# Hyungi-Lee/Scale-Mixtures-of-Neural-Network-Gaussian-Processes

Measured on AMD Instinct MI355X. Metric: kernel-build + Cholesky wallclock (ms) and GFLOP/s at N=16384, 4-layer relu NNGP, higher is better.
Workload: dtype f32; 1 GPU; C4: SPR.loss = NNGP kernel build + jittered Cholesky + Gaussian LML, N=16384 d=3072 L=4 relu; N=16384, d=3072, layers=4, act=relu, parallelism=single GPU

## Files before the change

### include/smnngp.h

```cpp
#ifndef SMNNGP_H
#define SMNNGP_H

#include <stddef.h>
#include <stdint.h>

#ifdef __cplusplus
extern "C" {
#endif

typedef struct smn_ctx smn_ctx;

enum { SMN_OK = 0, SMN_EINVAL = -1, SMN_EHIP = -2, SMN_ENOMEM = -3, SMN_ENOTSUP = -4, SMN_ECOMM = -5 };
enum { SMN_F32 = 0, SMN_F64 = 1 };
enum { SMN_ACT_RELU = 0, SMN_ACT_ERF = 1 };
enum { SMN_GET_NNGP = 1, SMN_GET_NTK = 2 };
enum { SMN_FILL_FULL = 0, SMN_FILL_LOWER = 1 };
enum { SMN_NET_MLP = 0, SMN_NET_DENSE_RESNET = 1 };

int smn_version(void);
int smn_device_count(int* n);
int smn_ctx_create(int device_id, smn_ctx** out);
int smn_ctx_destroy(smn_ctx* ctx);
int smn_last_error(smn_ctx* ctx, char* buf, size_t n);
int smn_synchronize(smn_ctx* ctx);
// ... 62 lines not shown

int smn_trsm(smn_ctx* ctx, int dtype, const void* l_d, int64_t n, int64_t ldl,
             void* b_d, int64_t nrhs, int64_t ldb, int trans);
int smn_transpose(smn_ctx* ctx, int dtype, void* dst_d, int64_t ldd, const void* src_d, int64_t lds, int64_t rows,
                  int64_t cols);

int smn_lml(smn_ctx* ctx, int dtype, void* k_d, int64_t n, int64_t ldk, const void* y_d,
            double eps_abs, double df, double scale, double* logpdf_h, double* quad_h,
            double* logdet_h, int* info_h);

int smn_predict(smn_ctx* ctx, int dtype, void* kj_d, int64_t n, int64_t t, int64_t ldk,
                const void* y_d, int64_t c, double ridge_rel, double ridge_abs,
                void* mean_d, void* cov_d, int64_t ldcov, double* quad_h, double* logdet_h, int* info_h);

int smn_spr_loss(smn_ctx* ctx, int dtype, int net, int act, int num_hiddens,
                 double w_std, double b_std, double last_w_std,
                 const void* x_d, int64_t n, int64_t ldx, int64_t d, const void* y_d,
                 double eps_abs, double df, double scale,
                 double* logpdf_h, double* quad_h, double* logdet_h, int* info_h);
int smn_spr_predict(smn_ctx* ctx, int dtype, int net, int act, int num_hiddens,
                    double w_std, double b_std, double last_w_std,
                    const void* x_d, int64_t n, int64_t ldx, const void* xt_d, int64_t t, int64_t ldxt,
                    int64_t d, const void* y_d, int64_t c, double ridge_rel, double ridge_abs,
                    void* mean_d, void* cov_d, int64_t ldcov,
                    double* quad_h, double* logdet_h, int* info_h);

int smn_spr_loss_batch(smn_ctx* ctx, int dtype, int net, int act, int num_hiddens, int nprob,
                       const double* w_std, const double* b_std, const double* last_w_std,
                       const void* x_d, int64_t n, int64_t ldx, int64_t d, const void* y_d,
                       const double* eps_abs, const double* df, const double* scale,
                       double* logpdf_h, double* quad_h, double* logdet_h, int* info_h);
int smn_debug_batch_bytes(smn_ctx* ctx, size_t bytes);
int smn_debug_split_build(smn_ctx* ctx, int on);
int smn_debug_gram_cache(smn_ctx* ctx, int on);
int smn_gram_cache_stats(smn_ctx* ctx, int64_t* hits, int64_t* misses, size_t* bytes);
int smn_debug_panel_passes(smn_ctx* ctx, int max_passes);
int smn_spr_predict_batch(smn_ctx* ctx, int dtype, int net, int act, int num_hiddens, int nprob,
                          const double* w_std, const double* b_std, const double* last_w_std,
                          const void* x_d, int64_t n, int64_t ldx, const void* xt_d, int64_t t, int64_t ldxt,
                          int64_t d, const void* y_d, int64_t c, const double* ridge_rel, const double* ridge_abs,
                          void* mean_d, void* cov_d, int64_t ldcov, void* var_d,
                          double* quad_h, double* logdet_h, int* info_h);

int smn_mixture_nll(smn_ctx* ctx, int dtype, int nprob, int64_t t, const void* mean_d, const void* var_d,
                    const double* quad_h, const double* logdet_h, const int* skip_h, const double* y_test_h,
                    double y_mean, double y_std, int64_t n, int nmix, int nsamples, const double* sample_q_h,
                    const double* ratio_h, double* tnll_h);

int smn_lml_grad_terms(smn_ctx* ctx, int dtype, int net, int act, int num_hiddens,
                       double w_std, double b_std, double last_w_std,
                       const void* k0_d, int64_t n, int64_t ldk0, const void* q_d,
                       const void* neg_kinv_d, int64_t ldkinv, const void* alpha_d,
                       double coef, double terms_h[4]);
int smn_spr_loss_grad(smn_ctx* ctx, int dtype, int net, int act, int num_hiddens,
                      double w_std, double b_std, double last_w_std,
                      const void* x_d, int64_t n, int64_t ldx, int64_t d, const void* y_d,
                      double eps_abs, double df, double scale,
                      double* quad_h, double* logdet_h, int* info_h, double terms_h[4]);
int smn_spr_loss_grad_batch(smn_ctx* ctx, int dtype, int net, int act, int num_hiddens, int nprob,
                            const double* w_std, const double* b_std, const double* last_w_std,
                            const void* x_d, int64_t n, int64_t ldx, int64_t d, const void* y_d,
                            const double* eps_abs, const double* df, const double* scale,
                            double* quad_h, double* logdet_h, int* info_h, double* terms_h);

#define SMN_CNN_GRAD_MAX_PIXELS 1024
int smn_kernel_cnn_grad_terms(smn_ctx* ctx, int dtype, int act, int num_hiddens,
// ... 71 lines not shown
```

### scale-mixtures-of-neural-network-gaussian-processes_amd/_lib.py

```python
from __future__ import annotations

import ctypes as C
import os

import numpy as np

_HERE = os.path.dirname(os.path.abspath(__file__))
LIB_PATH = os.environ.get("SMNNGP_LIB") or os.path.join(_HERE, "libsmnngp.so")

OK, EINVAL, EHIP, ENOMEM, ENOTSUP, ECOMM = 0, -1, -2, -3, -4, -5
F32, F64 = 0, 1
ACT = {"relu": 0, "erf": 1}
GET_NNGP, GET_NTK = 1, 2
FILL_FULL, FILL_LOWER = 0, 1
NET_MLP, NET_DENSE_RESNET = 0, 1


class SmnError(RuntimeError):
    def __init__(self, code, msg):
        super().__init__("libsmnngp error %d: %s" % (code, msg))
        self.code = code


def _load():
# ... 22 lines not shown
    "smn_free": [_vp, _vp],
    "smn_memset": [_vp, _vp, _i, _sz],
    "smn_memcpy_h2d": [_vp, _vp, _vp, _sz],
    "smn_memcpy_d2h": [_vp, _vp, _vp, _sz],
    "smn_memcpy_d2d": [_vp, _vp, _vp, _sz],
    "smn_memcpy2d_h2d": [_vp, _vp, _sz, _vp, _sz, _sz, _sz],
    "smn_memcpy2d_d2h": [_vp, _vp, _sz, _vp, _sz, _sz, _sz],
    "smn_timer_start": [_vp],
    "smn_timer_stop_ms": [_vp, _pd],
    "smn_profile_enable": [_vp, _i],
    "smn_profile_read": [_vp, _i, _pd, _pi],
    "smn_profile_flops": [_vp, _i, _pd],
    "smn_kernel_mlp": [_vp, _i, _i, _i, _i, _d, _d, _d, _vp, _i64, _i64, _vp, _i64, _i64, _i64, _i, _i, _vp, _vp, _i64],
    "smn_kernel_mlp_rows": [_vp, _i, _i, _i, _i, _d, _d, _d, _vp, _i64, _i64, _i64, _i64, _i64, _i, _vp, _vp, _i64],
    "smn_kernel_mlp_lower_rows": [_vp, _i, _i, _i, _i, _d, _d, _d, _vp, _i64, _i64, _i64, _i64, _i64, _i, _vp, _vp, _i64],
    "smn_kernel_mlp_shard": [_vp, _i, _i, _i, _i, _d, _d, _d, _vp, _i64, _i64, _i64, _i, _i, _i64, _i, _vp, _vp],
    "smn_gram": [_vp, _i, _vp, _i64, _i64, _vp, _i64, _i64, _i64, _vp, _i64, _vp, _vp],
    "smn_recursion": [_vp, _i, _i, _i, _i, _d, _d, _d, _vp, _i64, _i64, _i64, _vp, _vp, _i, _i, _vp, _vp, _i64],
    "smn_kernel_cnn": [_vp, _i, _i, _i, _d, _d, _d, _vp, _i64, _vp, _i64, _i64, _i64, _i64, _i, _vp, _i64],
    "smn_kernel_conv_resnet": [_vp, _i, _i, _i, _d, _d, _d, _vp, _i64, _vp, _i64, _i64, _i64, _i64, _i, _vp, _i64],
    "smn_cholesky": [_vp, _i, _vp, _i64, _i64, _i64, _i64, _d, _d, _pi, _pd],
    "smn_trsm": [_vp, _i, _vp, _i64, _i64, _vp, _i64, _i64, _i],
    "smn_transpose": [_vp, _i, _vp, _i64, _vp, _i64, _i64, _i64],
    "smn_lml": [_vp, _i, _vp, _i64, _i64, _vp, _d, _d, _d, _pd, _pd, _pd, _pi],
    "smn_predict": [_vp, _i, _vp, _i64, _i64, _i64, _vp, _i64, _d, _d, _vp, _vp, _i64, _pd, _pd, _pi],
    "smn_spr_loss": [_vp, _i, _i, _i, _i, _d, _d, _d, _vp, _i64, _i64, _i64, _vp, _d, _d, _d, _pd, _pd, _pd, _pi],
    "smn_spr_predict": [_vp, _i, _i, _i, _i, _d, _d, _d, _vp, _i64, _i64, _vp, _i64, _i64, _i64, _vp, _i64, _d, _d,
                        _vp, _vp, _i64, _pd, _pd, _pi],
    "smn_spr_loss_batch": [_vp, _i, _i, _i, _i, _i, _pd, _pd, _pd, _vp, _i64, _i64, _i64, _vp, _pd, _pd, _pd, _pd, _pd, _pd, _pi],
    "smn_spr_predict_batch": [_vp, _i, _i, _i, _i, _i, _pd, _pd, _pd, _vp, _i64, _i64, _vp, _i64, _i64, _i64, _vp, _i64, _pd, _pd,
                              _vp, _vp, _i64, _vp, _pd, _pd, _pi],
    "smn_debug_batch_bytes": [_vp, _sz],
    "smn_debug_split_build": [_vp, C.c_int],
    "smn_debug_gram_cache": [_vp, C.c_int],
    "smn_gram_cache_stats": [_vp, C.POINTER(C.c_int64), C.POINTER(C.c_int64), C.POINTER(C.c_size_t)],
    "smn_debug_panel_passes": [_vp, C.c_int],
    "smn_mixture_nll": [_vp, _i, _i, _i64, _vp, _vp, _pd, _pd, _pi, _pd, _d, _d, _i64, _i, _i, _pd, _pd, _pd],
    "smn_comm_unique_id": [C.c_char_p],
    "smn_lml_grad_terms": [_vp, _i, _i, _i, _i, _d, _d, _d, _vp, _i64, _i64, _vp, _vp, _i64, _vp, _d, _pd],
    "smn_spr_loss_grad": [_vp, _i, _i, _i, _i, _d, _d, _d, _vp, _i64, _i64, _i64, _vp, _d, _d, _d, _pd, _pd, _pi, _pd],
    "smn_spr_loss_grad_batch": [_vp, _i, _i, _i, _i, _i, _pd, _pd, _pd, _vp, _i64, _i64, _i64, _vp, _pd, _pd, _pd, _pd, _pd, _pi, _pd],
    "smn_kernel_cnn_grad_terms": [_vp, _i, _i, _i, _d, _d, _d, _vp, _i64, _i64, _i64, _i64, _vp, _i64, _vp, _d, _pd],
    "smn_spr_cnn_loss_grad": [_vp, _i, _i, _i, _d, _d, _d, _vp, _i64, _i64, _i64, _i64, _vp, _d, _d, _d, _pd, _pd, _pi, _pd],
    "smn_kernel_conv_diag": [_vp, _i, _i, _i, _i, _d, _d, _d, _vp, _i64, _i64, _i64, _i64, _vp],
    "smn_svsp_moments": [_vp, _i, _vp, _vp, _vp, _vp, _vp, _i64, _i64, _i64, _d, _vp, _vp, _pi, _pi64],
    "smn_mc_softmax": [_vp, _i, _vp, _vp, _pi, _i64, _i64, _i64, _d, C.c_uint64, _i64, _vp, _vp, _vp, _vp],
    "smn_rng_variates": [_vp, _i, C.c_uint64, _d, _i64, _i64, _i64, _i64, _vp],
    "smn_rng_variates_ddf": [_vp, _i, C.c_uint64, _d, _i64, _i64, _i64, _i64, _vp, _vp],
    "smn_svsp_head_grad": [_vp, _i, _vp, _vp, _pi, _i64, _i64, _i64, _d, _d, C.c_uint64, _i64, _vp, _vp, _pd, _vp, _vp, _pd, _pd, _pi],
    "smn_svsp_elbo_grad": [_vp, _i, _vp, _i64, _i64, _i64, _i64, _vp, _vp, _d, _d, _d, _pi, _i64, _d, _d, C.c_uint64, _i64, _vp, _vp,
                           _pd, _pd, _vp, _vp, _pd, _pd, _pd, _pd, _vp, _i64, _pi],
    "smn_debug_philox": [_vp, C.POINTER(C.c_uint32), C.POINTER(C.c_uint32), C.POINTER(C.c_uint32)],
    "smn_comm_init": [_vp, _i, _i, C.c_char_p],
    "smn_comm_destroy": [_vp],
    "smn_allgather": [_vp, _i, _i, _vp, _vp, _i64],
    "smn_unpack_lower_blocks": [_vp, _i, _vp, _i64, _i, _i64, _vp, _i64],
    "smn_lml_from_blocks": [_vp, _i, _vp, _i64, _i, _i64, _vp, _d, _d, _d, _pd, _pd, _pd, _pi],
    "smn_comm_info": [_vp, _pi, _pi],
    "smn_shard_begin": [_vp, _i, _i64, _d],
    "smn_kernel_mlp_shard_cols": [_vp, _i, _i, _i, _i, _d, _d, _d, _vp, _i64, _i64, _i64, _i, _i, _i, _pi64, _i, _vp, _vp],
    "smn_shard_exchange_cols": [_vp, _i, _vp, _vp, _i64, _i, _i, _pi64, _i],
    "smn_shard_exchange_cols_to": [_vp, _i, _vp, _vp, _i64, _i, _i, _pi64, _i, _vp, _i64],
    "smn_shard_scatter_cols": [_vp, _i, _vp, _i64, _i, _i, _pi64, _i, _vp, _i64],
    "smn_shard_wait": [_vp],
    "smn_lml_from_shards": [_vp, _i, _i64, _vp, _d, _d, _pd, _pd, _pd, _pi],
    "smn_debug_delay": [_vp, _i, _i64],
# ... 200 lines not shown
```

### scale-mixtures-of-neural-network-gaussian-processes_amd/csrc/api.hip

```cpp
#include <climits>

#include "internal.hpp"

int smn_allow_lds(smn_ctx* ctx, const void* kernel, size_t lds) {
  size_t& have = ctx->max_lds[kernel];
  if (lds <= have) return SMN_OK;
  SMN_HIP(ctx, hipFuncSetAttribute(kernel, hipFuncAttributeMaxDynamicSharedMemorySize, (int)lds));
  have = lds;
  return SMN_OK;
}

static int sync_side_streams(smn_ctx* ctx) {
  if (ctx->stream_comm) SMN_HIP(ctx, hipStreamSynchronize(ctx->stream_comm));
  if (ctx->stream_scatter) SMN_HIP(ctx, hipStreamSynchronize(ctx->stream_scatter));
  if (ctx->stream_bulk) SMN_HIP(ctx, hipStreamSynchronize(ctx->stream_bulk));
  return SMN_OK;
}

int smn_workspace(smn_ctx* ctx, int slot, size_t bytes, void** out) {
  if (slot < 0 || slot >= smn_ctx::kSlots) return smn_fail(ctx, SMN_EINVAL, "bad workspace slot");
  if (ctx->ws_bytes[slot] < bytes) {
    if (slot == 2) {
      ctx->shard_a = nullptr;
      ctx->arrivals.clear();
// ... 231 lines not shown
extern "C" int smn_ctx_create(int device_id, smn_ctx** out) {
  if (!out) return SMN_EINVAL;
  *out = nullptr;
  int cnt = 0;
  if (hipGetDeviceCount(&cnt) != hipSuccess || cnt <= 0 || device_id < 0 || device_id >= cnt) return SMN_EHIP;
  if (hipSetDevice(device_id) != hipSuccess) return SMN_EHIP;
  smn_ctx* c = new smn_ctx();
  c->device = device_id;
  if (const char* e = getenv("SMN_XCD_MAP")) c->xcd_map = e[0] == '1';
  if (const char* e = getenv("SMN_SUPER")) c->super_panel = atol(e);
  if (const char* e = getenv("SMN_SUPER_WIDE_ROWS")) c->super_wide_rows = atol(e);
  if (const char* e = getenv("SMN_PANEL_LEAF")) c->panel_leaf = e[0] != '0';
  {
    hipDeviceProp_t prop;
    if (hipGetDeviceProperties(&prop, device_id) == hipSuccess && prop.multiProcessorCount > 0)
      c->num_cu = prop.multiProcessorCount;
  }
  int prio_lo = 0, prio_hi = 0;
  (void)hipDeviceGetStreamPriorityRange(&prio_lo, &prio_hi);
  auto masked_stream = [&](hipStream_t* st, int lo, int hi) -> bool {
    uint32_t mask[8] = {0, 0, 0, 0, 0, 0, 0, 0};
    for (int b = lo; b < hi && b < 256; ++b) mask[b >> 5] |= 1u << (b & 31);
    return hipExtStreamCreateWithCUMask(st, 8, mask) == hipSuccess;
  };
  const bool main_ok = hipStreamCreateWithPriority(&c->stream, hipStreamNonBlocking, prio_hi) == hipSuccess;
  if (const char* e = getenv("SMN_CHAIN_CUS")) c->chain_cus = atoi(e);
  if (const char* e = getenv("SMN_CHAIN_MIN_N")) c->chain_min_n = atol(e);
  if (c->chain_cus > 0 && c->chain_cus < c->num_cu) {
    if (!masked_stream(&c->stream_bulk, c->chain_cus, c->num_cu)) c->stream_bulk = nullptr;
  }
  bool ok = main_ok &&
            hipEventCreateWithFlags(&c->ev_a, hipEventDisableTiming) == hipSuccess &&
            hipEventCreateWithFlags(&c->ev_b, hipEventDisableTiming) == hipSuccess &&
            hipEventCreateWithFlags(&c->ev_c0, hipEventDisableTiming) == hipSuccess &&
            hipEventCreateWithFlags(&c->ev_c1, hipEventDisableTiming) == hipSuccess &&
            hipStreamCreateWithPriority(&c->stream_comm, hipStreamNonBlocking, prio_hi) == hipSuccess &&
            hipStreamCreateWithPriority(&c->stream_scatter, hipStreamNonBlocking, prio_hi) == hipSuccess &&
            hipEventCreate(&c->ev_t0) == hipSuccess && hipEventCreate(&c->ev_t1) == hipSuccess &&
            hipMalloc(reinterpret_cast<void**>(&c->d_scal), 64 * sizeof(double)) == hipSuccess &&
            hipMalloc(reinterpret_cast<void**>(&c->d_info), 16 * sizeof(int)) == hipSuccess &&
            hipHostMalloc(reinterpret_cast<void**>(&c->h_mail), smn_ctx::kMailDoubles * sizeof(double), hipHostMallocMapped) == hipSuccess &&
            hipHostGetDevicePointer(reinterpret_cast<void**>(&c->d_mail), c->h_mail, 0) == hipSuccess;
  if (!ok) {
    smn_ctx_destroy(c);
    return SMN_EHIP;
  }
  c->h_mail[smn_ctx::kMailGram] = 0.0;
  *out = c;
  return SMN_OK;
}

extern "C" int smn_ctx_destroy(smn_ctx* c) {
  if (!c) return SMN_OK;
  (void)hipSetDevice(c->device);
  if (c->stream_bulk) (void)hipStreamSynchronize(c->stream_bulk);
  if (c->stream_comm) (void)hipStreamSynchronize(c->stream_comm);
  if (c->stream_scatter) (void)hipStreamSynchronize(c->stream_scatter);
  if (c->stream) (void)hipStreamSynchronize(c->stream);
  if (c->comm) smn_comm_destroy(c);
  gram_cache_drop(c, true);
  if (c->gram.word) (void)hipFree(c->gram.word);
  for (int i = 0; i < smn_ctx::kSlots; ++i)
    if (c->ws[i]) (void)hipFree(c->ws[i]);
  for (hipEvent_t e : c->prof_ev) (void)hipEventDestroy(e);
  if (c->d_scal) (void)hipFree(c->d_scal);
  if (c->d_info) (void)hipFree(c->d_info);
  if (c->h_mail) (void)hipHostFree(c->h_mail);
  if (c->ev_a) (void)hipEventDestroy(c->ev_a);
  if (c->ev_b) (void)hipEventDestroy(c->ev_b);
  if (c->ev_s0) (void)hipEventDestroy(c->ev_s0);
  if (c->ev_corner) (void)hipEventDestroy(c->ev_corner);
  if (c->tile_list) (void)hipFree(c->tile_list);
  if (c->ev_c0) (void)hipEventDestroy(c->ev_c0);
  if (c->ev_c1) (void)hipEventDestroy(c->ev_c1);
  if (c->stream_comm) (void)hipStreamDestroy(c->stream_comm);
  if (c->stream_scatter) (void)hipStreamDestroy(c->stream_scatter);
  for (hipEvent_t e : c->ev_pool) (void)hipEventDestroy(e);
  if (c->ev_t0) (void)hipEventDestroy(c->ev_t0);
  if (c->ev_t1) (void)hipEventDestroy(c->ev_t1);
  if (c->stream) (void)hipStreamDestroy(c->stream);
  if (c->stream_bulk) (void)hipStreamDestroy(c->stream_bulk);
  delete c;
  return SMN_OK;
}

extern "C" int smn_last_error(smn_ctx* ctx, char* buf, size_t n) {
  if (!ctx || !buf || n == 0) return SMN_EINVAL;
  snprintf(buf, n, "%s", ctx->err.c_str());
  return SMN_OK;
}

extern "C" int smn_synchronize(smn_ctx* ctx) {
  if (!ctx) return SMN_EINVAL;
  SMN_ENTER(ctx);
  SMN_HIP(ctx, hipStreamSynchronize(ctx->stream));
  return SMN_OK;
}

extern "C" int smn_malloc(smn_ctx* ctx, size_t bytes, void** dptr) {
  if (!ctx || !dptr) return SMN_EINVAL;
  SMN_ENTER(ctx);
  *dptr = nullptr;
// ... 118 lines not shown
```

### scale-mixtures-of-neural-network-gaussian-processes_amd/csrc/cholesky.hip

```cpp
#include <climits>
#include <cstdlib>
#include <type_traits>
#include <vector>

#include "gemm_nt.hpp"
#include "internal.hpp"
#include "panel_leaf.hpp"

namespace {

constexpr int PB = 128;
constexpr int MP = 8;
constexpr int kQuarterTileMax = 256;
constexpr int kHalfTileMax = 384;
constexpr int kPersistMaxK = 512;
constexpr int kPanelSmallRows = 4096;
constexpr int kPanelSmallXR = 16;
constexpr int64_t kSuperWide = 2048;
constexpr int64_t kOuterWide = 512;
constexpr int64_t kF0FirstTiles = 2000;

template <typename T>
struct PanelCfg;
#ifndef SMN_PANEL_XR
#define SMN_PANEL_XR 128
#endif
template <>
struct PanelCfg<float> {
  static constexpr int XR = SMN_PANEL_XR;
  static constexpr int LD = PB + 4;
};
template <>
struct PanelCfg<double> {
  static constexpr int XR = 16;
  static constexpr int LD = PB + 2;
};
template <typename T>
struct PanelMma;
template <>
struct PanelMma<float> {
  static constexpr int TM = 16, ACC = 4, KSTEP = 16, NK = 4;
  using acc_t = f32x4;
  using vec_t = f32x4;
  static __device__ __forceinline__ int frag_row(int lane) { return lane & 15; }
  static __device__ __forceinline__ int frag_k(int lane) { return (lane >> 4) * 4; }
  static __device__ __forceinline__ void mma1(acc_t& c, float a, float b) {
    c = __builtin_amdgcn_mfma_f32_16x16x4f32(a, b, c, 0, 0, 0);
  }
  static __device__ __forceinline__ int acc_row(int lane, int i) { return 4 * (lane >> 4) + i; }
  static __device__ __forceinline__ int acc_col(int lane) { return lane & 15; }
};
template <>
struct PanelMma<double> {
// ... 857 lines not shown
  }
}

template <typename T>
__global__ void diag_trace_kernel(const T* __restrict__ a, int64_t lda, int64_t n, double* __restrict__ out) {
  __shared__ double red[256];
  double s = 0.0;
  for (int64_t i = threadIdx.x; i < n; i += 256) s += (double)a[i * lda + i];
  red[threadIdx.x] = s;
  __syncthreads();
  for (int o = 128; o > 0; o >>= 1) {
    if ((int)threadIdx.x < o) red[threadIdx.x] += red[threadIdx.x + o];
    __syncthreads();
  }
  if (threadIdx.x == 0) *out = red[0];
}

template <typename T>
__global__ void diag_shift_kernel(T* __restrict__ a, int64_t lda, int64_t n, double jitter_abs, double ridge_rel,
                                  const double* __restrict__ trace) {
  const int64_t i = (int64_t)blockIdx.x * blockDim.x + threadIdx.x;
  if (i >= n) return;
  const double sh = jitter_abs + (ridge_rel != 0.0 ? ridge_rel * (*trace) / (double)n : 0.0);
  a[i * lda + i] = (T)((double)a[i * lda + i] + sh);
}

__global__ void init_scalars_kernel(double* logdet, int* info) {
  *logdet = 0.0;
  *info = INT_MAX;
}

template <typename T>
int launch_update(smn_ctx* ctx, const FactorCall& f, hipStream_t st, T* a, int64_t lda, int64_t r0, int64_t c0, int64_t k0,
                  int64_t K, int64_t tiles_m, int64_t tiles_n, int lower, int tag = -1) {
  if (tiles_m <= 0 || tiles_n <= 0 || K <= 0) return SMN_OK;
  if (tag < 0) tag = lower ? 1 : 0;
  if (f.id0 >= 0) {
    const int64_t id0 = f.id0, id1 = f.id1, r_end = r0 + tiles_m * kTile;
    const int64_t act = std::min(id1, id0 + (k0 + K + kTile - 1) / kTile * kTile);
    if (act < id1 && r_end > act) {
      FactorCall live = f;
      live.id0 = live.id1 = -1;
      if (r0 < act) SMN_TRY(launch_update<T>(ctx, live, st, a, lda, r0, c0, k0, K, (act - r0) / kTile, tiles_n, lower, tag));
      if (r_end > id1) {
        const int64_t tb = (r_end - id1) / kTile;
        const int64_t nb = lower == 1 ? (act - c0) / kTile : tiles_n;
        SMN_TRY(launch_update<T>(ctx, live, st, a, lda, id1, c0, k0, K, tb, nb, 0, tag));
        if (lower == 1) SMN_TRY(launch_update<T>(ctx, live, st, a, lda, id1, id1, k0, K, tb, tb, 1, tag));
      }
      return SMN_OK;
    }
  }
  if (lower == 2 && tiles_n >= tiles_m) {
    lower = 1;
    tiles_n = tiles_m;
  }
  UpdArgs<T> u{a, lda, r0, c0, k0, (int)K, (int)tiles_n, lower, 0, TileMap::make(tiles_m, tiles_n, lower == 1),
               f.batch_logdet ? f.batch_stride : 0};
  const unsigned gy = (unsigned)(f.batch_logdet ? f.batch : 1);
  int64_t nt = lower == 1   ? tiles_m * (tiles_m + 1) / 2
               : lower == 2 ? tiles_n * (tiles_n + 1) / 2 + (tiles_m - tiles_n) * tiles_n
                            : tiles_m * tiles_n;
  ctx->prof_flops[tag ? PROF_TRAIL : PROF_STRIP] += 2.0 * kTile * kTile * (double)K * (double)nt * gy;
  if (ctx->xcd_map && nt >= 512 && lower != 2) {
    u.use_map = 1;
    nt = u.map.grid;
  }
  const size_t lds = MainTile<T>::LDS_BYTES;
  if constexpr (sizeof(T) == 4) {
    const int cus = (st == ctx->stream_bulk && st != nullptr) ? ctx->num_cu - ctx->chain_cus : ctx->num_cu;
    if (tag == 1 && lower && !u.use_map && gy == 1 && nt > 2 * cus && K <= kPersistMaxK) {
      const size_t plds = TileNT<T, kTile, kTile, 2>::LDS_BYTES;
      ProfScope ps(ctx, PROF_TRAIL, st);
      hipLaunchKernelGGL(trail_kernel<T>, dim3((unsigned)(2 * cus)), dim3(256), plds, st, u, (int)nt);
      SMN_CHECK_LAUNCH(ctx);
      return SMN_OK;
    }
  }
  if (!u.use_map && nt <= kQuarterTileMax) {
    ProfScope ps(ctx, tag ? PROF_TRAIL : PROF_STRIP, st);
    constexpr size_t qlds = TileNT<T, 64, 64, SMN_STAGES>::LDS_BYTES;
    if (tag) {
      auto kern = update_kernel<T, 1, 64, 64>;
      hipLaunchKernelGGL(kern, dim3((unsigned)(4 * nt), gy), dim3(256), qlds, st, u);
    } else {
      auto kern = update_kernel<T, 0, 64, 64>;
      hipLaunchKernelGGL(kern, dim3((unsigned)(4 * nt), gy), dim3(256), qlds, st, u);
    }
    SMN_CHECK_LAUNCH(ctx);
    return SMN_OK;
  }
  if (!u.use_map && nt <= kHalfTileMax) {
    const int64_t nh = lower == 1   ? tiles_m * (tiles_m + 1)
                       : lower == 2 ? tiles_n * (tiles_n + 1) + 2 * (tiles_m - tiles_n) * tiles_n
                                    : 2 * tiles_m * tiles_n;
    ProfScope ps(ctx, tag ? PROF_TRAIL : PROF_STRIP, st);
    constexpr size_t hlds = TileNT<T, 64, kTile, SMN_STAGES>::LDS_BYTES;
    if (tag) {
      auto kern = update_kernel<T, 1, 64>;
      hipLaunchKernelGGL(kern, dim3((unsigned)nh, gy), dim3(256), hlds, st, u);
    } else {
      auto kern = update_kernel<T, 0, 64>;
      hipLaunchKernelGGL(kern, dim3((unsigned)nh, gy), dim3(256), hlds, st, u);
    }
// ... 127 lines not shown
  }
  SMN_CHECK_LAUNCH(ctx);
  hipStream_t sb = (n_total >= ctx->chain_min_n && ctx->stream_bulk) ? ctx->stream_bulk : nullptr;
  const int64_t W = sb ? kOuterWide : 2 * PB;
  int64_t S = ctx->super_panel / W * W;
  if (S < W) S = W;
  int64_t Swide = kSuperWide;
  if (Swide < S) Swide = S;
  const bool noschur = f.noschur && n_factor < n_total;
  const bool arriving = f.n_arrivals > 0;
  std::vector<char> seen_main, seen_bulk;
  if (arriving) {
    seen_main.assign(f.n_arrivals, 0);
    seen_bulk.assign(f.n_arrivals, 0);
  }
  bool first_need = true;
  auto need_columns = [&](hipStream_t s, int64_t col_hi) -> int {
    if (!arriving) return SMN_OK;
    std::vector<char>& seen = (s == st) ? seen_main : seen_bulk;
    bool any = false;
    for (size_t i = 0; i < f.n_arrivals; ++i)
      if (!seen[i] && f.arrivals[i].col_begin < col_hi) any = true;
    if (!any) return SMN_OK;
    ProfScope ps(ctx, first_need ? PROF_EXPOSED : PROF_STALL, s);
    first_need = false;
    for (size_t i = 0; i < f.n_arrivals; ++i)
      if (!seen[i] && f.arrivals[i].col_begin < col_hi) {
        SMN_HIP(ctx, hipStreamWaitEvent(s, f.arrivals[i].ev, 0));
        seen[i] = 1;
      }
    return SMN_OK;
  };
  auto width = [&](int64_t c0) { return (sb && n_total - c0 >= ctx->super_wide_rows) ? Swide : S; };
  for (int64_t s0 = 0, s_stop = 0; s0 < n_factor; s0 = s_stop) {
    const int64_t Sc = width(s0);
    const int64_t s_end = (n_factor - s0 < Sc) ? n_factor : s0 + Sc;
    s_stop = s_end;
    for (int64_t j0 = s0; j0 < s_end; j0 += W) {
      const int64_t w = (s_end - j0 < W) ? s_end - j0 : W;
      for (int64_t js = j0; js < j0 + w; js += PB) {
        SMN_TRY(need_columns(st, js + PB));
        if (js > j0)
          SMN_TRY(launch_update<T>(ctx, f, st, a, lda, js, js, j0, js - j0, (n_total - js) / kTile, 1, 0));
        SMN_TRY(launch_panel<T>(ctx, f, st, a, lda, js, n_total, 0));
      }
      const int64_t j1 = j0 + w;
      if (j1 < s_end) SMN_TRY(need_columns(st, s_end));
      if (j1 < s_end)
        SMN_TRY(launch_update<T>(ctx, f, st, a, lda, j1, j1, j0, w, (n_total - j1) / kTile, (s_end - j1) / kTile, 2));
    }
    if (s_end >= n_total) break;
    const int64_t K = s_end - s0;
    if (!sb) {
      SMN_TRY(need_columns(st, n_total));
      const int64_t tm = (n_total - s_end) / kTile;
      if (!noschur) SMN_TRY(launch_update<T>(ctx, f, st, a, lda, s_end, s_end, s0, K, tm, tm, 1));
      else if (n_factor > s_end) SMN_TRY(launch_update<T>(ctx, f, st, a, lda, s_end, s_end, s0, K, tm, (n_factor - s_end) / kTile, 2));
      continue;
    }
    const int64_t Sn = width(s_end);
    const int64_t s_next = s_end >= n_factor ? s_end : ((n_factor - s_end < Sn) ? n_factor : s_end + Sn);
    const int64_t tm1 = n_total > s_next ? (n_total - s_next) / kTile : 0;
    const int64_t tn1 = noschur ? (n_factor > s_next ? (n_factor - s_next) / kTile : 0) : tm1;
    const bool f0_first = tn1 * (tn1 + 1) / 2 + (tm1 - tn1) * tn1 <= kF0FirstTiles;
    if (!f0_first) {
      SMN_HIP(ctx, hipEventRecord(ctx->ev_a, st));
      SMN_HIP(ctx, hipStreamWaitEvent(sb, ctx->ev_a, 0));
    }
    if (bulk.side) SMN_HIP(ctx, hipStreamWaitEvent(st, ctx->ev_b, 0));
    if (s_next > s_end) SMN_TRY(need_columns(st, s_next));
    if (s_next > s_end)
      SMN_TRY(launch_update<T>(ctx, f, st, a, lda, s_end, s_end, s0, K, (n_total - s_end) / kTile, (s_next - s_end) / kTile, 2));
    if (f0_first) {
      SMN_HIP(ctx, hipEventRecord(ctx->ev_a, st));
      SMN_HIP(ctx, hipStreamWaitEvent(sb, ctx->ev_a, 0));
    }
    if (n_total > s_next && tn1 > 0) {
      const int64_t tm = (n_total - s_next) / kTile;
      bulk.side = sb;
      SMN_TRY(need_columns(sb, n_total));
      if (!noschur) {
        SMN_TRY(launch_update<T>(ctx, f, sb, a, lda, s_next, s_next, s0, K, tm, tm, 1));
      } else {
        SMN_TRY(launch_update<T>(ctx, f, sb, a, lda, s_next, s_next, s0, K, tn1, tn1, 1));
        if (tm > tn1) SMN_TRY(launch_update<T>(ctx, f, sb, a, lda, s_next + tn1 * kTile, s_next, s0, K, tm - tn1, tn1, 0, 1));
      }
      SMN_HIP(ctx, hipEventRecord(ctx->ev_b, sb));
    }
  }
  SMN_TRY(need_columns(st, INT64_MAX));
  pieces.release();
  SMN_TRY(bulk.join());
  if (f.keep_factor && f.batch_logdet) return smn_fail(ctx, SMN_ENOTSUP, "cholesky: keep_factor in a batched factorisation");
  if (f.keep_factor) {
    hipLaunchKernelGGL(copy_diag_kernel<T>, dim3((unsigned)(n_factor / PB)), dim3(1024), 0, st, a, lda,
                       static_cast<const T*>(side));
    SMN_CHECK_LAUNCH(ctx);
  }
  return SMN_OK;
}

}

int inverse_from_rows(smn_ctx* ctx, int dtype, const void* x, int64_t ldx, const void* z, int64_t kcols, int64_t n,
                      void* neg_inv, int64_t ldo, void* alpha, double* quad_dev) {
  const int64_t t = (n + kTile - 1) / kTile, ntiles = t * (t + 1) / 2;
  if (dtype == SMN_F64) SMN_TRY(set_lds_attrs<double>(ctx)); else SMN_TRY(set_lds_attrs<float>(ctx));
  {
    ProfScope ps(ctx, PROF_TRAIL, ctx->stream);
    ctx->prof_flops[PROF_TRAIL] += 2.0 * kTile * kTile * (double)kTile * (double)(t * (t + 1) * (t + 2) / 6);
    if (dtype == SMN_F64) {
      SMN_TRY(smn_allow_lds(ctx, reinterpret_cast<const void*>(syrk_rows_kernel<double>), MainTile<double>::LDS_BYTES));
// ... 110 lines not shown
```

### scale-mixtures-of-neural-network-gaussian-processes_amd/csrc/common.hpp

```cpp
#pragma once
#include <hip/hip_runtime.h>

#include <cstdarg>
#include <cstdint>
#include <cstdio>
#include <cstdlib>
#include <cstring>
#include <string>
#include <unordered_map>
#include <vector>

#include "../../include/smnngp.h"

struct smn_ctx {
  int device = 0;
  hipStream_t stream = nullptr;
  hipStream_t stream_bulk = nullptr;
  int chain_cus = 32;
  int64_t chain_min_n = 8192;
  hipStream_t stream_comm = nullptr;
  hipStream_t stream_scatter = nullptr;
  hipEvent_t ev_a = nullptr, ev_b = nullptr, ev_t0 = nullptr, ev_t1 = nullptr;
  hipEvent_t ev_c0 = nullptr, ev_c1 = nullptr;
  void* shard_a = nullptr; int64_t shard_lda = 0, shard_n = 0; int shard_dtype = -1; double shard_eps = 0.0;
  struct Arrival { int64_t col_begin, col_end; hipEvent_t ev; };
  std::vector<Arrival> arrivals;
  std::vector<hipEvent_t> ev_pool;
  size_t ev_pool_used = 0;
  std::string err;
  static constexpr int kSlots = 12;
  void* ws[kSlots] = {};
  size_t ws_bytes[kSlots] = {};
  double* d_scal = nullptr;
  int* d_info = nullptr;
  double* h_mail = nullptr;
  double* d_mail = nullptr;
  static constexpr int kMailGram = 64, kMailDoubles = 72;
  void* comm = nullptr;
  int nranks = 1, rank = 0;
  bool prof = false;
  unsigned prof_mask = ~0u;
  std::vector<hipEvent_t> prof_ev;
  std::vector<int> prof_cat;
  size_t prof_used = 0;
  double prof_flops[12] = {};
  int num_cu = 256;
  int64_t super_panel = 1024;
  int64_t super_wide_rows = 18432;
  size_t batch_bytes = (size_t)48 << 30;
  int* tile_list = nullptr; int64_t tile_list_cap = 0; int tile_list_tm = 0, tile_list_tb = 0, tile_list_na = 0, tile_list_nb = 0;
  hipEvent_t ev_s0 = nullptr, ev_corner = nullptr;
  bool split_build = true;
  int panel_max_passes = 4;
  std::unordered_map<const void*, size_t> max_lds;
  bool lds_attrs_done[2] = {false, false};
// ... 105 lines not shown
```

### scale-mixtures-of-neural-network-gaussian-processes_amd/csrc/heads.hip

```cpp
#include <algorithm>
#include <climits>
#include <cmath>
#include <vector>

#include "internal.hpp"

namespace {

struct Aug {
  int64_t n, n_pad, t, c, n_total, lda;
  void* a;
  size_t es;
  char* at(int64_t r, int64_t col) const { return static_cast<char*>(a) + es * (size_t)(r * lda + col); }
};

int aug_alloc(smn_ctx* ctx, int dtype, int64_t n, int64_t t, int64_t c, Aug* g) {
  g->n = n; g->t = t; g->c = c;
  g->n_pad = round_up(n, kTile);
  g->n_total = g->n_pad + round_up(t + c, kTile);
  g->lda = g->n_total;
  g->es = dtype_size(dtype);
  return smn_workspace(ctx, 2, g->es * (size_t)g->n_total * (size_t)g->n_total, &g->a);
}

// ... 646 lines not shown
      else
        hipLaunchKernelGGL(batch_extract_kernel<float>, ge, dim3(256), 0, ctx->stream, static_cast<const float*>(g.a), g.lda, bstride, g.n_pad, t, c,
                           reinterpret_cast<float*>(mean_p), reinterpret_cast<float*>(cov_p), ldcov, reinterpret_cast<float*>(var_p), res_d, ld_d, info_d);
    }
    SMN_CHECK_LAUNCH(ctx);
    SMN_HIP(ctx, hipMemcpyAsync(res_h.data(), res_d, sizeof(double) * (size_t)nb * (2 + (size_t)c), hipMemcpyDeviceToHost, ctx->stream));
    SMN_HIP(ctx, hipStreamSynchronize(ctx->stream));
    for (int b = 0; b < nb; ++b) {
      const double* r = &res_h[(size_t)b * (2 + (size_t)c)];
      int info = (int)r[1];
      if (info == INT_MAX) info = 0;
      if (info_h) info_h[p0 + b] = info;
      if (logdet_h) logdet_h[p0 + b] = info ? std::nan("") : r[0];
      for (int64_t k = 0; k < c && quad_h; ++k) quad_h[(size_t)(p0 + b) * (size_t)c + (size_t)k] = info ? std::nan("") : r[2 + k];
    }
  }
  return SMN_OK;
}

}

extern "C" int smn_debug_panel_passes(smn_ctx* ctx, int max_passes) {
  if (!ctx || max_passes < 1 || max_passes > 64) return SMN_EINVAL;
  ctx->panel_max_passes = max_passes;
  return SMN_OK;
}

extern "C" int smn_debug_split_build(smn_ctx* ctx, int on) {
  if (!ctx) return SMN_EINVAL;
  ctx->split_build = on != 0;
  return SMN_OK;
}

extern "C" int smn_debug_gram_cache(smn_ctx* ctx, int on) {
  if (!ctx) return SMN_EINVAL;
  SMN_ENTER(ctx);
  ctx->gram.enabled = on != 0;
  if (!ctx->gram.enabled) gram_cache_drop(ctx, true);
  return SMN_OK;
}

extern "C" int smn_gram_cache_stats(smn_ctx* ctx, int64_t* hits, int64_t* misses, size_t* bytes) {
  if (!ctx) return SMN_EINVAL;
  if (hits) *hits = ctx->gram.hits;
  if (misses) *misses = ctx->gram.misses;
  if (bytes) *bytes = ctx->gram.xc_bytes + ctx->gram.g0_bytes;
  return SMN_OK;
}

extern "C" int smn_debug_batch_bytes(smn_ctx* ctx, size_t bytes) {
  if (!ctx || bytes == 0) return SMN_EINVAL;
  ctx->batch_bytes = bytes;
  return SMN_OK;
}

extern "C" int smn_spr_loss_batch(smn_ctx* ctx, int dtype, int net, int act, int num_hiddens, int nprob, const double* w_std,
                                  const double* b_std, const double* last_w_std, const void* x_d, int64_t n, int64_t ldx,
                                  int64_t d, const void* y_d, const double* eps_abs, const double* df, const double* scale,
                                  double* logpdf_h, double* quad_h, double* logdet_h, int* info_h) {
  if (!ctx || !x_d || !y_d) return SMN_EINVAL;
  SMN_ENTER(ctx);
  if (nprob <= 0 || !eps_abs) return smn_fail(ctx, SMN_EINVAL, "smn_spr_loss_batch: empty batch or null eps_abs");
  for (int b = 0; b < nprob && df; ++b)
    if (df[b] > 0.0 && !(scale && scale[b] > 0.0)) return smn_fail(ctx, SMN_EINVAL, "smn_spr_loss_batch: scale must be > 0");
  std::vector<double> quad((size_t)nprob), ld((size_t)nprob);
  std::vector<int> info((size_t)nprob);
// ... 45 lines not shown
```

Baseline: 208,900 GFLOP/s.

## Eagerly apply next super-panel F0 update on bulk stream during panel chain

While the current super-panel's outer panels are still being factored on the main stream, each finished outer block's rank-w update is applied to the next super-panel's columns on the bulk stream. By the end of the super-panel, only the remaining K slice of the F0 update is left on the critical path. Eager mode is gated by a threshold on the previous F1 tile count and can be switched by a debug setter. The change adds event dependencies and competes for CUs with the chain and the F1 work. It also disables the persistent trail kernel for partial F0 launches.

```diff
diff --git a/include/smnngp.h b/include/smnngp.h
--- a/include/smnngp.h
+++ b/include/smnngp.h
@@ -118,6 +118,7 @@
                        double* logpdf_h, double* quad_h, double* logdet_h, int* info_h);
 int smn_debug_batch_bytes(smn_ctx* ctx, size_t bytes);
 int smn_debug_split_build(smn_ctx* ctx, int on);
+int smn_debug_eager_f0(smn_ctx* ctx, int mode);
 int smn_debug_gram_cache(smn_ctx* ctx, int on);
 int smn_gram_cache_stats(smn_ctx* ctx, int64_t* hits, int64_t* misses, size_t* bytes);
 int smn_debug_panel_passes(smn_ctx* ctx, int max_passes);
diff --git a/scale-mixtures-of-neural-network-gaussian-processes_amd/_lib.py b/scale-mixtures-of-neural-network-gaussian-processes_amd/_lib.py
--- a/scale-mixtures-of-neural-network-gaussian-processes_amd/_lib.py
+++ b/scale-mixtures-of-neural-network-gaussian-processes_amd/_lib.py
@@ -78,6 +78,7 @@
                               _vp, _vp, _i64, _vp, _pd, _pd, _pi],
     "smn_debug_batch_bytes": [_vp, _sz],
     "smn_debug_split_build": [_vp, C.c_int],
+    "smn_debug_eager_f0": [_vp, C.c_int],
     "smn_debug_gram_cache": [_vp, C.c_int],
     "smn_gram_cache_stats": [_vp, C.POINTER(C.c_int64), C.POINTER(C.c_int64), C.POINTER(C.c_size_t)],
     "smn_debug_panel_passes": [_vp, C.c_int],
diff --git a/scale-mixtures-of-neural-network-gaussian-processes_amd/csrc/api.hip b/scale-mixtures-of-neural-network-gaussian-processes_amd/csrc/api.hip
--- a/scale-mixtures-of-neural-network-gaussian-processes_amd/csrc/api.hip
+++ b/scale-mixtures-of-neural-network-gaussian-processes_amd/csrc/api.hip
@@ -287,6 +287,8 @@
   bool ok = main_ok &&
             hipEventCreateWithFlags(&c->ev_a, hipEventDisableTiming) == hipSuccess &&
             hipEventCreateWithFlags(&c->ev_b, hipEventDisableTiming) == hipSuccess &&
+            hipEventCreateWithFlags(&c->ev_e0, hipEventDisableTiming) == hipSuccess &&
+            hipEventCreateWithFlags(&c->ev_e1, hipEventDisableTiming) == hipSuccess &&
             hipEventCreateWithFlags(&c->ev_c0, hipEventDisableTiming) == hipSuccess &&
             hipEventCreateWithFlags(&c->ev_c1, hipEventDisableTiming) == hipSuccess &&
             hipStreamCreateWithPriority(&c->stream_comm, hipStreamNonBlocking, prio_hi) == hipSuccess &&
@@ -323,6 +325,8 @@
   if (c->h_mail) (void)hipHostFree(c->h_mail);
   if (c->ev_a) (void)hipEventDestroy(c->ev_a);
   if (c->ev_b) (void)hipEventDestroy(c->ev_b);
+  if (c->ev_e0) (void)hipEventDestroy(c->ev_e0);
+  if (c->ev_e1) (void)hipEventDestroy(c->ev_e1);
   if (c->ev_s0) (void)hipEventDestroy(c->ev_s0);
   if (c->ev_corner) (void)hipEventDestroy(c->ev_corner);
   if (c->tile_list) (void)hipFree(c->tile_list);
diff --git a/scale-mixtures-of-neural-network-gaussian-processes_amd/csrc/cholesky.hip b/scale-mixtures-of-neural-network-gaussian-processes_amd/csrc/cholesky.hip
--- a/scale-mixtures-of-neural-network-gaussian-processes_amd/csrc/cholesky.hip
+++ b/scale-mixtures-of-neural-network-gaussian-processes_amd/csrc/cholesky.hip
@@ -19,6 +19,10 @@
 constexpr int64_t kSuperWide = 2048;
 constexpr int64_t kOuterWide = 512;
 constexpr int64_t kF0FirstTiles = 2000;
+#ifndef SMN_EAGER_F0_TILES
+#define SMN_EAGER_F0_TILES 3000
+#endif
+constexpr int64_t kEagerF0Tiles = SMN_EAGER_F0_TILES;
 
 template <typename T>
 struct PanelCfg;
@@ -942,7 +946,7 @@
 
 template <typename T>
 int launch_update(smn_ctx* ctx, const FactorCall& f, hipStream_t st, T* a, int64_t lda, int64_t r0, int64_t c0, int64_t k0,
-                  int64_t K, int64_t tiles_m, int64_t tiles_n, int lower, int tag = -1) {
+                  int64_t K, int64_t tiles_m, int64_t tiles_n, int lower, int tag = -1, bool persist = true) {
   if (tiles_m <= 0 || tiles_n <= 0 || K <= 0) return SMN_OK;
   if (tag < 0) tag = lower ? 1 : 0;
   if (f.id0 >= 0) {
@@ -951,12 +955,12 @@
     if (act < id1 && r_end > act) {
       FactorCall live = f;
       live.id0 = live.id1 = -1;
-      if (r0 < act) SMN_TRY(launch_update<T>(ctx, live, st, a, lda, r0, c0, k0, K, (act - r0) / kTile, tiles_n, lower, tag));
+      if (r0 < act) SMN_TRY(launch_update<T>(ctx, live, st, a, lda, r0, c0, k0, K, (act - r0) / kTile, tiles_n, lower, tag, persist));
       if (r_end > id1) {
         const int64_t tb = (r_end - id1) / kTile;
         const int64_t nb = lower == 1 ? (act - c0) / kTile : tiles_n;
-        SMN_TRY(launch_update<T>(ctx, live, st, a, lda, id1, c0, k0, K, tb, nb, 0, tag));
-        if (lower == 1) SMN_TRY(launch_update<T>(ctx, live, st, a, lda, id1, id1, k0, K, tb, tb, 1, tag));
+        SMN_TRY(launch_update<T>(ctx, live, st, a, lda, id1, c0, k0, K, tb, nb, 0, tag, persist));
+        if (lower == 1) SMN_TRY(launch_update<T>(ctx, live, st, a, lda, id1, id1, k0, K, tb, tb, 1, tag, persist));
       }
       return SMN_OK;
     }
@@ -979,7 +983,7 @@
   const size_t lds = MainTile<T>::LDS_BYTES;
   if constexpr (sizeof(T) == 4) {
     const int cus = (st == ctx->stream_bulk && st != nullptr) ? ctx->num_cu - ctx->chain_cus : ctx->num_cu;
-    if (tag == 1 && lower && !u.use_map && gy == 1 && nt > 2 * cus && K <= kPersistMaxK) {
+    if (persist && tag == 1 && lower && !u.use_map && gy == 1 && nt > 2 * cus && K <= kPersistMaxK) {
       const size_t plds = TileNT<T, kTile, kTile, 2>::LDS_BYTES;
       ProfScope ps(ctx, PROF_TRAIL, st);
       hipLaunchKernelGGL(trail_kernel<T>, dim3((unsigned)(2 * cus)), dim3(256), plds, st, u, (int)nt);
@@ -1173,10 +1177,17 @@
     return SMN_OK;
   };
   auto width = [&](int64_t c0) { return (sb && n_total - c0 >= ctx->super_wide_rows) ? Swide : S; };
+  bool have_f1 = false;
+  int64_t prev_f1_tiles = 0;
   for (int64_t s0 = 0, s_stop = 0; s0 < n_factor; s0 = s_stop) {
     const int64_t Sc = width(s0);
     const int64_t s_end = (n_factor - s0 < Sc) ? n_factor : s0 + Sc;
     s_stop = s_end;
+    const int64_t Sn = width(s_end);
+    const int64_t s_next = s_end >= n_factor ? s_end : ((n_factor - s_end < Sn) ? n_factor : s_end + Sn);
+    const bool eager = sb && s_next > s_end && ctx->eager_f0 != 0 &&
+                       (ctx->eager_f0 == 2 || s0 == 0 || prev_f1_tiles <= kEagerF0Tiles);
+    int64_t f0_k0 = s0;
     for (int64_t j0 = s0; j0 < s_end; j0 += W) {
       const int64_t w = (s_end - j0 < W) ? s_end - j0 : W;
       for (int64_t js = j0; js < j0 + w; js += PB) {
@@ -1186,6 +1197,15 @@
         SMN_TRY(launch_panel<T>(ctx, f, st, a, lda, js, n_total, 0));
       }
       const int64_t j1 = j0 + w;
+      if (eager && j1 < s_end) {
+        SMN_HIP(ctx, hipEventRecord(ctx->ev_e0, st));
+        bulk.side = sb;
+        SMN_TRY(need_columns(sb, s_next));
+        SMN_HIP(ctx, hipStreamWaitEvent(sb, ctx->ev_e0, 0));
+        SMN_TRY(launch_update<T>(ctx, f, sb, a, lda, s_end, s_end, j0, w, (n_total - s_end) / kTile, (s_next - s_end) / kTile, 2, -1, false));
+        f0_k0 = j1;
+        if (j1 + W >= s_end) SMN_HIP(ctx, hipEventRecord(ctx->ev_e1, sb));
+      }
       if (j1 < s_end) SMN_TRY(need_columns(st, s_end));
       if (j1 < s_end)
         SMN_TRY(launch_update<T>(ctx, f, st, a, lda, j1, j1, j0, w, (n_total - j1) / kTile, (s_end - j1) / kTile, 2));
@@ -1199,8 +1219,6 @@
       else if (n_factor > s_end) SMN_TRY(launch_update<T>(ctx, f, st, a, lda, s_end, s_end, s0, K, tm, (n_factor - s_end) / kTile, 2));
       continue;
     }
-    const int64_t Sn = width(s_end);
-    const int64_t s_next = s_end >= n_factor ? s_end : ((n_factor - s_end < Sn) ? n_factor : s_end + Sn);
     const int64_t tm1 = n_total > s_next ? (n_total - s_next) / kTile : 0;
     const int64_t tn1 = noschur ? (n_factor > s_next ? (n_factor - s_next) / kTile : 0) : tm1;
     const bool f0_first = tn1 * (tn1 + 1) / 2 + (tm1 - tn1) * tn1 <= kF0FirstTiles;
@@ -1208,17 +1226,21 @@
       SMN_HIP(ctx, hipEventRecord(ctx->ev_a, st));
       SMN_HIP(ctx, hipStreamWaitEvent(sb, ctx->ev_a, 0));
     }
-    if (bulk.side) SMN_HIP(ctx, hipStreamWaitEvent(st, ctx->ev_b, 0));
+    if (f0_k0 > s0) SMN_HIP(ctx, hipStreamWaitEvent(st, ctx->ev_e1, 0));
+    else if (have_f1) SMN_HIP(ctx, hipStreamWaitEvent(st, ctx->ev_b, 0));
     if (s_next > s_end) SMN_TRY(need_columns(st, s_next));
     if (s_next > s_end)
-      SMN_TRY(launch_update<T>(ctx, f, st, a, lda, s_end, s_end, s0, K, (n_total - s_end) / kTile, (s_next - s_end) / kTile, 2));
+      SMN_TRY(launch_update<T>(ctx, f, st, a, lda, s_end, s_end, f0_k0, s_end - f0_k0, (n_total - s_end) / kTile, (s_next - s_end) / kTile, 2, -1,
+                               f0_k0 == s0));
     if (f0_first) {
       SMN_HIP(ctx, hipEventRecord(ctx->ev_a, st));
       SMN_HIP(ctx, hipStreamWaitEvent(sb, ctx->ev_a, 0));
     }
+    prev_f1_tiles = tn1 * (tn1 + 1) / 2 + (tm1 - tn1) * tn1;
     if (n_total > s_next && tn1 > 0) {
       const int64_t tm = (n_total - s_next) / kTile;
       bulk.side = sb;
+      have_f1 = true;
       SMN_TRY(need_columns(sb, n_total));
       if (!noschur) {
         SMN_TRY(launch_update<T>(ctx, f, sb, a, lda, s_next, s_next, s0, K, tm, tm, 1));
diff --git a/scale-mixtures-of-neural-network-gaussian-processes_amd/csrc/common.hpp b/scale-mixtures-of-neural-network-gaussian-processes_amd/csrc/common.hpp
--- a/scale-mixtures-of-neural-network-gaussian-processes_amd/csrc/common.hpp
+++ b/scale-mixtures-of-neural-network-gaussian-processes_amd/csrc/common.hpp
@@ -21,6 +21,8 @@
   hipStream_t stream_comm = nullptr;
   hipStream_t stream_scatter = nullptr;
   hipEvent_t ev_a = nullptr, ev_b = nullptr, ev_t0 = nullptr, ev_t1 = nullptr;
+  hipEvent_t ev_e0 = nullptr, ev_e1 = nullptr;
+  int eager_f0 = 1;
   hipEvent_t ev_c0 = nullptr, ev_c1 = nullptr;
   void* shard_a = nullptr; int64_t shard_lda = 0, shard_n = 0; int shard_dtype = -1; double shard_eps = 0.0;
   struct Arrival { int64_t col_begin, col_end; hipEvent_t ev; };
diff --git a/scale-mixtures-of-neural-network-gaussian-processes_amd/csrc/heads.hip b/scale-mixtures-of-neural-network-gaussian-processes_amd/csrc/heads.hip
--- a/scale-mixtures-of-neural-network-gaussian-processes_amd/csrc/heads.hip
+++ b/scale-mixtures-of-neural-network-gaussian-processes_amd/csrc/heads.hip
@@ -702,6 +702,12 @@
   return SMN_OK;
 }
 
+extern "C" int smn_debug_eager_f0(smn_ctx* ctx, int mode) {
+  if (!ctx || mode < 0 || mode > 2) return SMN_EINVAL;
+  ctx->eager_f0 = mode;
+  return SMN_OK;
+}
+
 extern "C" int smn_debug_gram_cache(smn_ctx* ctx, int on) {
   if (!ctx) return SMN_EINVAL;
   SMN_ENTER(ctx);
diff --git a/scratch/r10/chain_timeline.py b/scratch/r10/chain_timeline.py
--- /dev/null
+++ b/scratch/r10/chain_timeline.py
@@ -0,0 +1,112 @@
+import argparse
+import collections
+import csv
+import glob
+import os
+import re
+
+p = argparse.ArgumentParser()
+p.add_argument("trace")
+p.add_argument("--n-total", type=int, default=16512)
+p.add_argument("--threshold", type=int, default=4000)
+p.add_argument("--super", type=int, default=1024)
+p.add_argument("--outer", type=int, default=512)
+p.add_argument("--warmup", type=int, default=3)
+args = p.parse_args()
+PB = 128
+TAG1 = re.compile(r"trail_kernel|update_kernel<\w+, 1")
+f = max(glob.glob(args.trace + "/**/*kernel_trace.csv", recursive=True), key=os.path.getsize)
+rows = list(csv.DictReader(open(f)))
+
+
+def short(n):
+    return n.replace("void (anonymous namespace)::", "").split("(")[0]
+
+
+ks = sorted((int(r["Start_Timestamp"]), int(r["End_Timestamp"]), short(r["Kernel_Name"]), r["Queue_Id"]) for r in rows)
+starts = [i for i, k in enumerate(ks) if k[2].startswith("pad_rows_kernel")]
+steps = [ks[a:b] for a, b in zip(starts, starts[1:] + [len(ks)])]
+n_sp = (args.n_total - PB + args.super - 1) // args.super
+per_sp, per_outer = args.super // PB, args.outer // PB
+
+
+def f1_tiles(s):
+    tm = max(0, (args.n_total - min((s + 2) * args.super, args.n_total - PB)) // PB)
+    return tm * (tm + 1) // 2
+
+
+eager_rule = [s for s in range(n_sp - 1) if s == 0 or f1_tiles(s - 1) <= args.threshold]
+
+
+def analyse(step):
+    qs = collections.Counter(k[3] for k in step if "panelr_kernel" in k[2])
+    mainq = max(qs, key=qs.get)
+    upd = lambda k: k[2].startswith(("update_kernel", "trail_kernel"))
+    main = [k for k in step if k[3] == mainq]
+    bulk = [k for k in step if k[3] != mainq and upd(k)]
+    sp, cur, np_ = [], None, 0
+    for k in main:
+        if k[2].startswith("panelr_kernel"):
+            if np_ % per_sp == 0:
+                cur = {"panels": [], "f0": None}
+                sp.append(cur)
+            cur["panels"].append(k)
+            np_ += 1
+        elif cur is not None and len(cur["panels"]) == per_sp and cur["f0"] is None and TAG1.match(k[2]):
+            cur["f0"] = k
+    for s, c in enumerate(sp):
+        c["beg"], c["end"] = c["panels"][0][0], c["panels"][-1][1]
+        c["ready"] = [c["panels"][i][1] for i in range(per_outer - 1, len(c["panels"]) - 1, per_outer)]
+        c["E"] = [b for b in bulk if c["ready"] and c["ready"][0] <= b[0] < c["end"]]
+    taken = {id(b) for c in sp for b in c["E"]}
+    f1 = [b for b in bulk if id(b) not in taken]
+    for s, c in enumerate(sp):
+        hi = sp[s + 1]["end"] if s + 1 < len(sp) else 1 << 62
+        c["F1"] = [b for b in f1 if c["end"] <= b[0] < hi]
+    return sp
+
+
+def sum_f0(sp, which):
+    return sum((sp[s]["f0"][1] - sp[s]["f0"][0]) for s in which if s < len(sp) and sp[s]["f0"]) / 1e6
+
+
+timed = steps[args.warmup:]
+vals = [sum_f0(analyse(st), eager_rule) for st in timed]
+allf0 = [sum_f0(analyse(st), range(n_sp)) for st in timed]
+span = [(max(k[1] for k in st) - st[0][0]) / 1e6 for st in timed]
+print("trace %s: %d steps, %d timed" % (args.trace, len(steps), len(timed)))
+print("eager super-panels under the rule (threshold %d tiles): %s" % (args.threshold, eager_rule))
+print("sum F0 over those, ms per step: mean %.3f (min %.3f max %.3f); over every super-panel: mean %.3f" %
+      (sum(vals) / len(vals), min(vals), max(vals), sum(allf0) / len(allf0)))
+print("kernel span of a step (first start to last end), ms: mean %.3f min %.3f max %.3f" % (sum(span) / len(span), min(span), max(span)))
+step = steps[-1]
+sp = analyse(step)
+t0 = step[0][0]
+ms = lambda t: (t - t0) / 1e6
+print("last step: span %.3f ms" % ms(max(k[1] for k in step)))
+print("%3s | %8s %8s | %-26s | %-17s | %8s %8s %6s %7s | %s" % ("s", "chain beg", "end", "eager pieces start-end (ready)", "F1(s-1) start-end", "F0 start", "end", "ms", "gap", "F0 waited for"))
+for s, c in enumerate(sp):
+    e = " ".join("%.3f-%.3f" % (ms(b[0]), ms(b[1])) for b in c["E"]) or "-"
+    if c["E"]:
+        e += " (%.3f)" % ms(c["ready"][0])
+    pf = sp[s - 1]["F1"] if s else []
+    f1s = "%.3f-%.3f" % (ms(pf[0][0]), ms(pf[-1][1])) if pf else "-"
+    if c["f0"]:
+        k = c["f0"]
+        cands = {"chain": c["end"]}
+        if c["E"]:
+            cands["piece"] = max(b[1] for b in c["E"])
+        if pf:
+            cands["F1(s-1)"] = pf[-1][1]
+        who = max(cands, key=cands.get)
+        f0 = "%8.3f %8.3f %6.3f %7.3f | %s" % (ms(k[0]), ms(k[1]), (k[1] - k[0]) / 1e6, (k[0] - c["end"]) / 1e6, who)
+    else:
+        f0 = "-"
+    print("%3d | %8.3f %8.3f | %-26s | %-17s | %s" % (s, ms(c["beg"]), ms(c["end"]), e, f1s, f0))
+cnt = collections.defaultdict(lambda: [0, 0.0])
+mainq = sp[0]["panels"][0][3]
+for k in step:
+    cnt[("main " if k[3] == mainq else "bulk ") + k[2]][0] += 1
+    cnt[("main " if k[3] == mainq else "bulk ") + k[2]][1] += (k[1] - k[0]) / 1e6
+for n, v in sorted(cnt.items(), key=lambda kv: -kv[1][1])[:12]:
+    print("  %-50s x%-4d %.3f ms" % (n[:50], v[0], v[1]))
```

Result: no change. 209,700 GFLOP/s (median of 6 runs) (+0.4%).
